# smyers119/sdrtrunk

Measured on NVIDIA B200. Metric: channelized+demodulated complex MS/s and real-time channel count at 1/2/4/8 GPU, higher is better.
Workload: dtype f32

## Files before the change

sdrtrunk_b200/csrc/filters.cu:

```cuda
#include <cstdint>

#include "filters.cuh"
#include "tma.cuh"

using namespace sdrgpu;

namespace {

__global__ void halfband_kernel(const float2 *__restrict__ in, long long in_stride, float2 *__restrict__ out,
                                long long out_stride, int out_off, int n_out, const __grid_constant__ HalfBandTaps taps)
{
    const int c = blockIdx.y;
    const float2 *x = in + (size_t)c * in_stride;
    float2 *y = out + (size_t)c * out_stride + out_off;
    const int L = taps.length, half = (L - 1) / 2;
    for (int m = blockIdx.x * blockDim.x + threadIdx.x; m < n_out; m += gridDim.x * blockDim.x) {
        const float2 *p = x + 2 * m;
        float ai = 0.0f, aq = 0.0f;
        for (int j = 0; j < half; j += 2) {
            const float2 a = p[j], b = p[L - 1 - j];
            const float h = taps.c[j];
            ai = __fadd_rn(ai, __fmul_rn(h, __fadd_rn(a.x, b.x)));
            aq = __fadd_rn(aq, __fmul_rn(h, __fadd_rn(a.y, b.y)));
        }
        const float2 mid = p[half];
        ai = __fadd_rn(ai, __fmul_rn(mid.x, 0.5f));
        aq = __fadd_rn(aq, __fmul_rn(mid.y, 0.5f));
        y[m] = make_float2(ai, aq);
    }
}

constexpr int kFirThreads = 128;
constexpr int kFirPer = 8;

__device__ __forceinline__ int skew8(int i) { return i + 2 * (i >> 3); }

__host__ __device__ inline int fir_window_len(int window) { return (window + 2 * (window >> 3) + 8 + 1) & ~1; }

__device__ __forceinline__ float agc_envelope(float i, float q)
{
    const float a = fabsf(i), b = fabsf(q);
    return (a > b) ? __fadd_rn(a, __fmul_rn(0.4f, b)) : __fadd_rn(b, __fmul_rn(0.4f, a));
}

__device__ __forceinline__ void load8p(const float2 *group, float2 *w)
{
    const float4 *p = reinterpret_cast<const float4 *>(group);
#pragma unroll
    for (int q = 0; q < 4; q++) {
        const float4 v = p[q];
        w[2 * q] = make_float2(v.x, v.y);
        w[2 * q + 1] = make_float2(v.z, v.w);
    }
}

__device__ __forceinline__ void cp_async16(void *dst_shared, const void *src_global)
{
    asm volatile("cp.async.cg.shared.global [%0], [%1], 16;" ::"r"((uint32_t)__cvta_generic_to_shared(dst_shared)), "l"(src_global) : "memory");
}
__device__ __forceinline__ void cp_async_commit() { asm volatile("cp.async.commit_group;" ::: "memory"); }
template <int kPending>
__device__ __forceinline__ void cp_async_wait() { asm volatile("cp.async.wait_group %0;" ::"n"(kPending) : "memory"); }

__device__ __forceinline__ void fir_taps8(const float2 *wbase, const float *hs, int kp, float2 (&acc)[kFirPer])
{
    float2 ga[8], gb[8], gc[8];
    load8p(wbase, gc);
    load8p(wbase - 10, gb);
#pragma unroll
    for (int j = 0; j < kFirPer; j++) acc[j] = make_float2(0.0f, 0.0f);
#define FIR_STEP(lo, hi, k0_)                                                                                   \
    {                                                                                                           \
        const float4 ha_ = *reinterpret_cast<const float4 *>(hs + (k0_));                                       \
        const float4 hb_ = *reinterpret_cast<const float4 *>(hs + (k0_) + 4);                                   \
        const float h_[8] = {ha_.x, ha_.y, ha_.z, ha_.w, hb_.x, hb_.y, hb_.z, hb_.w};                           \
        _Pragma("unroll") for (int u = 0; u < 8; u++) {                                                         \
            const float2 hh_ = make_float2(h_[u], h_[u]);                                                       \
            _Pragma("unroll") for (int j = 0; j < kFirPer; j++) {                                               \
                const float2 x_ = (j - u >= 0) ? hi[j - u] : lo[8 + j - u];                                     \
                acc[j] = __ffma2_rn(x_, hh_, acc[j]);                                                           \
            }                                                                                                   \
        }                                                                                                       \
    }
    int k0 = 0;
    for (; k0 + 24 <= kp; k0 += 24, wbase -= 30) {
        load8p(wbase - 20, ga);
        FIR_STEP(gb, gc, k0);
        load8p(wbase - 30, gc);
        FIR_STEP(ga, gb, k0 + 8);
        if (k0 + 24 < kp) load8p(wbase - 40, gb);
        FIR_STEP(gc, ga, k0 + 16);
    }
    if (k0 < kp) {
        if (k0 + 8 < kp) load8p(wbase - 20, ga);
        FIR_STEP(gb, gc, k0);
        if (k0 + 8 < kp) FIR_STEP(ga, gb, k0 + 8);
    }
#undef FIR_STEP
}

__global__ void __launch_bounds__(kFirThreads)
fir_agc_kernel(const float2 *__restrict__ in, long long in_stride, int in_off, float2 *__restrict__ out,
               long long out_stride, int tile, int n_total, int kp, float fir_gain, int agc, int tiles_per_cta,
               const __grid_constant__ FirTaps taps)
{
    extern __shared__ __align__(16) float2 xs_all[];
    __shared__ __align__(16) float hs[kMaxFirTaps];
    __shared__ float red[kFirThreads / 32];
    const int c = blockIdx.y, tid = threadIdx.x;
    const int window = kp + ((tile + 7) & ~7);
    const int wlen = fir_window_len(window);
    const int n_tiles = (n_total + tile - 1) / tile;
    const int first = blockIdx.x * tiles_per_cta, last = min(first + tiles_per_cta, n_tiles);
    const float2 *row = in + (size_t)c * in_stride + in_off;
    auto fill = [&](int blk, float2 *xs) {
        const float2 *src = row + (size_t)blk * tile - kp;
        const int valid = kp + min(tile, n_total - blk * tile);
        if (valid == window) {
            const float2 *s = src + 2 * tid;
            float2 *d = xs + skew8(2 * tid);
            for (int i = 2 * tid; i < window; i += 2 * kFirThreads, s += 2 * kFirThreads, d += 2 * kFirThreads + (kFirThreads >> 1))
                cp_async16(d, s);
        } else {
            for (int i = 2 * tid; i < window; i += 2 * kFirThreads) {
                float2 *dst = xs + skew8(i);
                if (i + 1 < valid) {
                    cp_async16(dst, src + i);
                } else {
                    dst[0] = i < valid ? src[i] : make_float2(0.f, 0.f);
                    dst[1] = make_float2(0.f, 0.f);
                }
            }
        }
        cp_async_commit();
    };
    for (int k = tid; k < kp; k += kFirThreads) hs[k] = taps.h[k];
    if (first < last) fill(first, xs_all);
    for (int blk = first; blk < last; blk++) {
    float2 *xs = xs_all + ((blk - first) & 1) * wlen;
    if (blk + 1 < last) {
        fill(blk + 1, xs_all + (((blk - first) & 1) ^ 1) * wlen);
        cp_async_wait<1>();
    } else {
        cp_async_wait<0>();
    }
    __syncthreads();
    const int block = min(tile, n_total - blk * tile);

    const int n0 = tid * kFirPer;
    float ai[kFirPer], aq[kFirPer];
    if (n0 < block) {
        const float2 *wbase = xs + skew8(kp + n0);
        if (kp > 0) {
            float2 acc[kFirPer];
            fir_taps8(wbase, hs, kp, acc);
#pragma unroll
            for (int j = 0; j < kFirPer; j++) {
                ai[j] = __fmul_rn(acc[j].x, fir_gain);
                aq[j] = __fmul_rn(acc[j].y, fir_gain);
            }
        } else {
            float2 x[kFirPer];
            load8p(wbase, x);
#pragma unroll
            for (int j = 0; j < kFirPer; j++) {
                ai[j] = x[j].x;
                aq[j] = x[j].y;
            }
        }
    } else {
#pragma unroll
        for (int j = 0; j < kFirPer; j++) {
            ai[j] = 0.0f;
            aq[j] = 0.0f;
        }
    }

    if (agc) {
        float m = 0.0001f;
#pragma unroll
        for (int j = 0; j < kFirPer; j++) {
            if (n0 + j < block) {
                const float env = agc_envelope(ai[j], aq[j]);
                if (env > m) m = env;
            }
        }
#pragma unroll
        for (int o = 16; o > 0; o >>= 1) m = fmaxf(m, __shfl_xor_sync(0xffffffffu, m, o));
        if ((tid & 31) == 0) red[tid >> 5] = m;
        __syncthreads();
        m = red[0];
#pragma unroll
        for (int wdx = 1; wdx < kFirThreads / 32; wdx++) m = fmaxf(m, red[wdx]);
        const float g = __fdiv_rn(1.0f, m);
#pragma unroll
        for (int j = 0; j < kFirPer; j++) {
            ai[j] = __fmul_rn(ai[j], g);
            aq[j] = __fmul_rn(aq[j], g);
        }
    }
    float2 *dst = out + (size_t)c * out_stride + (size_t)blk * tile + n0;
    if (n0 + kFirPer <= block && ((reinterpret_cast<uintptr_t>(dst) & 15) == 0)) {
#pragma unroll
        for (int j = 0; j < kFirPer; j += 2) *reinterpret_cast<float4 *>(dst + j) = make_float4(ai[j], aq[j], ai[j + 1], aq[j + 1]);
    } else {
#pragma unroll
        for (int j = 0; j < kFirPer; j++)
            if (n0 + j < block) dst[j] = make_float2(ai[j], aq[j]);
    }
    __syncthreads();
    }
}

constexpr int kSplitTile = 1024;
constexpr int kSplitPerWarp = kSplitTile / (kFirThreads / 32);

__device__ __forceinline__ void mbar_arrive(uint64_t *bar)
{
    asm volatile("mbarrier.arrive.shared::cta.b64 _, [%0];" ::"r"(tma::smem_addr(bar)) : "memory");
}

__global__ void __launch_bounds__(kFirThreads, 5)
fir_agc_split_kernel(const float2 *__restrict__ in, long long in_stride, int in_off, float2 *__restrict__ out,
                     long long out_stride, int n_tiles, int kp, float fir_gain, int tiles_per_cta,
                     const __grid_constant__ FirTaps taps)
{
    extern __shared__ __align__(16) float2 xs_all[];
    __shared__ __align__(16) float hs[kMaxFirTaps];
    __shared__ float red[2][kFirThreads / 32];
    __shared__ __align__(8) uint64_t bars[2];
    const int c = blockIdx.y, tid = threadIdx.x, warp = tid >> 5, lane = tid & 31;
    const int window = kp + kSplitPerWarp;
    const int wlen = fir_window_len(window);
    const int first = blockIdx.x * tiles_per_cta, last = min(first + tiles_per_cta, n_tiles);
    if (first >= last) return;
    for (int k = tid; k < kp; k += kFirThreads) hs[k] = taps.h[k];
    if (tid == 0) {
        tma::mbar_init(&bars[0], kFirThreads / 32);
        tma::mbar_init(&bars[1], kFirThreads / 32);
    }
    __syncthreads();
    float2 *xw = xs_all + (size_t)warp * 2 * wlen;
    const float2 *row = in + (size_t)c * in_stride + in_off + warp * kSplitPerWarp - kp;
    float2 *orow = out + (size_t)c * out_stride + warp * kSplitPerWarp + lane * kFirPer;
    auto fill = [&](int blk, float2 *xs) {
        const float2 *s = row + (size_t)blk * kSplitTile + 2 * lane;
        float2 *d = xs + skew8(2 * lane);
        for (int i = 2 * lane; i < window; i += 64, s += 64, d += 80) cp_async16(d, s);
        cp_async_commit();
    };
    const float2 *wfirst = xw + skew8(kp + lane * kFirPer);
    float pi[kFirPer], pq[kFirPer];
    auto finish = [&](int t) {
        const int p = t & 1;
        tma::mbar_wait(&bars[p], (uint32_t)((t >> 1) & 1));
        float m = red[p][0];
#pragma unroll
        for (int wdx = 1; wdx < kFirThreads / 32; wdx++) m = fmaxf(m, red[p][wdx]);
        const float g = __fdiv_rn(1.0f, m);
        float2 *dst = orow + (size_t)(first + t) * kSplitTile;
        if ((reinterpret_cast<uintptr_t>(dst) & 15) == 0) {
#pragma unroll
            for (int j = 0; j < kFirPer; j += 2)
                *reinterpret_cast<float4 *>(dst + j) = make_float4(__fmul_rn(pi[j], g), __fmul_rn(pq[j], g), __fmul_rn(pi[j + 1], g), __fmul_rn(pq[j + 1], g));
        } else {
#pragma unroll
            for (int j = 0; j < kFirPer; j++) dst[j] = make_float2(__fmul_rn(pi[j], g), __fmul_rn(pq[j], g));
        }
    };
    fill(first, xw);
    for (int blk = first; blk < last; blk++) {
        const int t = blk - first, p = t & 1;
        if (blk + 1 < last) {
            fill(blk + 1, xw + (p ^ 1) * wlen);
            cp_async_wait<1>();
        } else {
            cp_async_wait<0>();
        }
        __syncwarp();
        float2 acc[kFirPer];
        fir_taps8(wfirst + p * wlen, hs, kp, acc);
        float ai[kFirPer], aq[kFirPer];
        float m = 0.0001f;
#pragma unroll
        for (int j = 0; j < kFirPer; j++) {
            ai[j] = __fmul_rn(acc[j].x, fir_gain);
            aq[j] = __fmul_rn(acc[j].y, fir_gain);
            const float env = agc_envelope(ai[j], aq[j]);
            if (env > m) m = env;
        }
        m = __uint_as_float(__reduce_max_sync(0xffffffffu, __float_as_uint(m)));
        if (t > 0) finish(t - 1);
        if (lane == 0) {
            red[p][warp] = m;
            mbar_arrive(&bars[p]);
        }
#pragma unroll
        for (int j = 0; j < kFirPer; j++) {
            pi[j] = ai[j];
            pq[j] = aq[j];
        }
        __syncwarp();
    }
    finish(last - 1 - first);
}

constexpr int kFirTilesPerCta = 4;

}

namespace sdrgpu {

sdrgpu_status halfband_launch(const float2 *in, long long in_stride, float2 *out, long long out_stride, int out_off,
                              int n_out, int n_channels, const HalfBandTaps &taps, cudaStream_t stream)
{
    dim3 grid((n_out + 255) / 256 > 64 ? 64 : (n_out + 255) / 256, n_channels);
    halfband_kernel<<<grid, 256, 0, stream>>>(in - (taps.length - 1), in_stride, out, out_stride, out_off, n_out, taps);
    count_launch();
    SDRGPU_CUDA(cudaGetLastError());
    return SDRGPU_OK;
}

sdrgpu_status fir_agc_launch(const FirLaunch &a)
{
    const int kp = fir_padded_taps(a.n_taps);
    const int tile = a.agc_block > 0 ? a.agc_block : (a.n < 1024 ? a.n : 1024);
    const size_t smem_need = sizeof(float2) * 2 * (size_t)fir_window_len(kp + ((tile + 7) & ~7));
    const size_t smem = (a.throttle || g_tuning[SDRGPU_TUNE_THROTTLE_ALWAYS]) ? smem_for_ctas_per_sm(smem_need, sizeof(float) * (kMaxFirTaps + 8), g_tuning[SDRGPU_TUNE_FIR_CTAS_PER_SM]) : smem_need;
    if (smem > 48 * 1024) {
        static size_t fir_attr = 0;
        if (smem > fir_attr) {
            SDRGPU_CUDA(cudaFuncSetAttribute(fir_agc_kernel, cudaFuncAttributeMaxDynamicSharedMemorySize, 226 * 1024 - (int)(sizeof(float) * (kMaxFirTaps + 8))));
            fir_attr = 226 * 1024;
        }
    }
    const int n_tiles = (a.n + tile - 1) / tile;
    int tpc = (int)(((long long)a.n_channels * n_tiles) / (148 * 12));
    tpc = tpc < 1 ? 1 : (tpc > kFirTilesPerCta ? kFirTilesPerCta : tpc);
    if (g_tuning[SDRGPU_TUNE_FIR_TILES_PER_CTA] > 0) tpc = g_tuning[SDRGPU_TUNE_FIR_TILES_PER_CTA];
    if (tpc > n_tiles) tpc = n_tiles;
    dim3 grid((n_tiles + tpc - 1) / tpc, a.n_channels);
    const size_t split_smem = sizeof(float2) * 2 * (kFirThreads / 32) * (size_t)fir_window_len(kp + kSplitPerWarp);
    if (a.agc_block > 0 && tile == kSplitTile && a.n % kSplitTile == 0 && kp >= 8 && smem == smem_need &&
        split_smem <= 48 * 1024 && (a.in_off & 1) == 0) {
        fir_agc_split_kernel<<<grid, kFirThreads, split_smem, a.stream>>>(a.in, a.in_stride, a.in_off, a.out, a.out_stride,
                                                                          n_tiles, kp, a.gain, tpc, *a.taps);
    } else {
        fir_agc_kernel<<<grid, kFirThreads, smem, a.stream>>>(a.in, a.in_stride, a.in_off, a.out, a.out_stride, tile, a.n, kp,
                                                              a.gain, a.agc_block > 0, tpc, *a.taps);
    }
    count_launch();
    SDRGPU_CUDA(cudaGetLastError());
    return SDRGPU_OK;
}

}
```

Baseline: 27310.

## Compute 16 FIR outputs per thread in split AGC kernel with smem staging

Generalizes the FIR tap loop into a templated ring-buffered routine and has the split FIR+AGC kernel compute 16 outputs per thread, using 2 warps per CTA instead of 4. Computed outputs are parked in a swizzled shared-memory buffer instead of registers, and the taps move into dynamic shared memory. The goal is more register-level reuse of loaded samples per tap and lower per-CTA overhead, with coalesced float4 stores in the finish step. The costs are higher register pressure, fewer warps per CTA for latency hiding, and a changed 16-sample skew layout that must stay consistent with the fill logic.

```diff
diff --git a/sdrtrunk_b200/csrc/filters.cu b/sdrtrunk_b200/csrc/filters.cu
--- a/sdrtrunk_b200/csrc/filters.cu
+++ b/sdrtrunk_b200/csrc/filters.cu
@@ -34,6 +34,10 @@
 constexpr int kFirPer = 8;
 
 __device__ __forceinline__ int skew8(int i) { return i + 2 * (i >> 3); }
+__device__ __forceinline__ int skew16(int i) { return i + 2 * (i >> 4); }
+
+template <int kOut>
+__host__ __device__ constexpr int fir_group_offset(int a) { return -8 * a - 2 * ((8 * a + 2 * kOut - 1) / kOut - 1); }
 
 __host__ __device__ inline int fir_window_len(int window) { return (window + 2 * (window >> 3) + 8 + 1) & ~1; }
 
@@ -62,40 +66,55 @@
 template <int kPending>
 __device__ __forceinline__ void cp_async_wait() { asm volatile("cp.async.wait_group %0;" ::"n"(kPending) : "memory"); }
 
-__device__ __forceinline__ void fir_taps8(const float2 *wbase, const float *hs, int kp, float2 (&acc)[kFirPer])
-{
-    float2 ga[8], gb[8], gc[8];
-    load8p(wbase, gc);
-    load8p(wbase - 10, gb);
-#pragma unroll
-    for (int j = 0; j < kFirPer; j++) acc[j] = make_float2(0.0f, 0.0f);
-#define FIR_STEP(lo, hi, k0_)                                                                                   \
+template <int kOut>
+__device__ __forceinline__ void fir_taps(const float2 *wbase, const float *hs, int kp, float2 (&acc)[kOut])
+{
+    static_assert(kOut % 8 == 0, "whole groups of 8 outputs");
+    constexpr int kRing = kOut / 8 + 2;
+    static_assert(kRing <= 4, "at most 16 outputs per thread");
+    float2 g[kRing][8];
+#pragma unroll
+    for (int a = 1 - kOut / 8; a <= 1; a++) load8p(wbase + fir_group_offset<kOut>(a), g[(a + kRing) % kRing]);
+#pragma unroll
+    for (int j = 0; j < kOut; j++) acc[j] = make_float2(0.0f, 0.0f);
+#define FIR_STEP(i_, k0_)                                                                                       \
     {                                                                                                           \
         const float4 ha_ = *reinterpret_cast<const float4 *>(hs + (k0_));                                       \
         const float4 hb_ = *reinterpret_cast<const float4 *>(hs + (k0_) + 4);                                   \
         const float h_[8] = {ha_.x, ha_.y, ha_.z, ha_.w, hb_.x, hb_.y, hb_.z, hb_.w};                           \
         _Pragma("unroll") for (int u = 0; u < 8; u++) {                                                         \
             const float2 hh_ = make_float2(h_[u], h_[u]);                                                       \
-            _Pragma("unroll") for (int j = 0; j < kFirPer; j++) {                                               \
-                const float2 x_ = (j - u >= 0) ? hi[j - u] : lo[8 + j - u];                                     \
-                acc[j] = __ffma2_rn(x_, hh_, acc[j]);                                                           \
+            _Pragma("unroll") for (int j = 0; j < kOut; j++) {                                                  \
+                const int d_ = j - u + 8;                                                                       \
+                acc[j] = __ffma2_rn(g[((i_) + 1 - d_ / 8 + kRing) % kRing][d_ % 8], hh_, acc[j]);               \
             }                                                                                                   \
         }                                                                                                       \
     }
+#define RING_STEP(i_)                                                                                           \
+    if constexpr ((i_) < kRing) {                                                                               \
+        if ((i_) + 1 < kRing || k0 + 8 * kRing < kp) load8p(wbase + fir_group_offset<kOut>((i_) + 2), g[((i_) + 2) % kRing]);   \
+        FIR_STEP(i_, k0 + 8 * (i_));                                                                            \
+    }
     int k0 = 0;
-    for (; k0 + 24 <= kp; k0 += 24, wbase -= 30) {
-        load8p(wbase - 20, ga);
-        FIR_STEP(gb, gc, k0);
-        load8p(wbase - 30, gc);
-        FIR_STEP(ga, gb, k0 + 8);
-        if (k0 + 24 < kp) load8p(wbase - 40, gb);
-        FIR_STEP(gc, ga, k0 + 16);
+    static_assert(8 * kRing % kOut == 0, "whole blocks per turn");
+    for (; k0 + 8 * kRing <= kp; k0 += 8 * kRing, wbase += fir_group_offset<kOut>(kRing)) {
+        RING_STEP(0)
+        RING_STEP(1)
+        RING_STEP(2)
+        RING_STEP(3)
+    }
+#undef RING_STEP
+#define TAIL_STEP(i_, more_)                                                                                    \
+    if constexpr ((i_) < kRing - 1) {                                                                           \
+        const bool next_ = (i_) + 1 < kRing - 1 && k0 + 8 * ((i_) + 1) < kp;                                    \
+        if ((i_) + 2 < kRing && next_) load8p(wbase + fir_group_offset<kOut>((i_) + 2), g[((i_) + 2) % kRing]);                  \
+        FIR_STEP(i_, k0 + 8 * (i_));                                                                            \
+        if (next_) { more_ }                                                                                    \
     }
     if (k0 < kp) {
-        if (k0 + 8 < kp) load8p(wbase - 20, ga);
-        FIR_STEP(gb, gc, k0);
-        if (k0 + 8 < kp) FIR_STEP(ga, gb, k0 + 8);
-    }
+        TAIL_STEP(0, TAIL_STEP(1, TAIL_STEP(2, )))
+    }
+#undef TAIL_STEP
 #undef FIR_STEP
 }
 
@@ -153,7 +172,7 @@
         const float2 *wbase = xs + skew8(kp + n0);
         if (kp > 0) {
             float2 acc[kFirPer];
-            fir_taps8(wbase, hs, kp, acc);
+            fir_taps<kFirPer>(wbase, hs, kp, acc);
 #pragma unroll
             for (int j = 0; j < kFirPer; j++) {
                 ai[j] = __fmul_rn(acc[j].x, fir_gain);
@@ -213,59 +232,75 @@
 }
 
 constexpr int kSplitTile = 1024;
-constexpr int kSplitPerWarp = kSplitTile / (kFirThreads / 32);
+constexpr int kSplitPer = 16;
+constexpr int kSplitWarps = kSplitTile / (32 * kSplitPer);
+constexpr int kSplitThreads = 32 * kSplitWarps;
+constexpr int kSplitPerWarp = kSplitTile / kSplitWarps;
+
+__host__ __device__ inline int fir_split_window_len(int kp) { return (((kp + 15) & ~15) + kSplitPerWarp) / 16 * 18; }
+
+inline size_t fir_split_smem(int kp)
+{
+    return sizeof(float) * kp + sizeof(float2) * kSplitWarps * (2 * (size_t)fir_split_window_len(kp) + kSplitPerWarp);
+}
 
 __device__ __forceinline__ void mbar_arrive(uint64_t *bar)
 {
     asm volatile("mbarrier.arrive.shared::cta.b64 _, [%0];" ::"r"(tma::smem_addr(bar)) : "memory");
 }
 
-__global__ void __launch_bounds__(kFirThreads, 5)
+__global__ void __launch_bounds__(kSplitThreads, 6)
 fir_agc_split_kernel(const float2 *__restrict__ in, long long in_stride, int in_off, float2 *__restrict__ out,
                      long long out_stride, int n_tiles, int kp, float fir_gain, int tiles_per_cta,
                      const __grid_constant__ FirTaps taps)
 {
     extern __shared__ __align__(16) float2 xs_all[];
-    __shared__ __align__(16) float hs[kMaxFirTaps];
-    __shared__ float red[2][kFirThreads / 32];
+    __shared__ float red[2][kSplitWarps];
     __shared__ __align__(8) uint64_t bars[2];
     const int c = blockIdx.y, tid = threadIdx.x, warp = tid >> 5, lane = tid & 31;
     const int window = kp + kSplitPerWarp;
-    const int wlen = fir_window_len(window);
+    const int kp16 = (kp + 15) & ~15;
+    const int wlen = fir_split_window_len(kp);
     const int first = blockIdx.x * tiles_per_cta, last = min(first + tiles_per_cta, n_tiles);
     if (first >= last) return;
-    for (int k = tid; k < kp; k += kFirThreads) hs[k] = taps.h[k];
+    float *hs = reinterpret_cast<float *>(xs_all);
+    for (int k = tid; k < kp; k += kSplitThreads) hs[k] = taps.h[k];
     if (tid == 0) {
-        tma::mbar_init(&bars[0], kFirThreads / 32);
-        tma::mbar_init(&bars[1], kFirThreads / 32);
+        tma::mbar_init(&bars[0], kSplitWarps);
+        tma::mbar_init(&bars[1], kSplitWarps);
     }
     __syncthreads();
-    float2 *xw = xs_all + (size_t)warp * 2 * wlen;
+    float2 *xw = xs_all + kp / 2 + (size_t)warp * (2 * wlen + kSplitPerWarp);
+    float4 *park = reinterpret_cast<float4 *>(xw + 2 * wlen);
     const float2 *row = in + (size_t)c * in_stride + in_off + warp * kSplitPerWarp - kp;
-    float2 *orow = out + (size_t)c * out_stride + warp * kSplitPerWarp + lane * kFirPer;
+    float2 *orow = out + (size_t)c * out_stride + warp * kSplitPerWarp;
     auto fill = [&](int blk, float2 *xs) {
         const float2 *s = row + (size_t)blk * kSplitTile + 2 * lane;
-        float2 *d = xs + skew8(2 * lane);
-        for (int i = 2 * lane; i < window; i += 64, s += 64, d += 80) cp_async16(d, s);
+        float2 *d = xs + skew16(kp16 - kp + 2 * lane);
+        for (int i = 2 * lane; i < window; i += 64, s += 64, d += 72) cp_async16(d, s);
         cp_async_commit();
     };
-    const float2 *wfirst = xw + skew8(kp + lane * kFirPer);
-    float pi[kFirPer], pq[kFirPer];
+    const float2 *wfirst = xw + skew16(kp16 + lane * kSplitPer);
     auto finish = [&](int t) {
         const int p = t & 1;
         tma::mbar_wait(&bars[p], (uint32_t)((t >> 1) & 1));
         float m = red[p][0];
 #pragma unroll
-        for (int wdx = 1; wdx < kFirThreads / 32; wdx++) m = fmaxf(m, red[p][wdx]);
+        for (int wdx = 1; wdx < kSplitWarps; wdx++) m = fmaxf(m, red[p][wdx]);
         const float g = __fdiv_rn(1.0f, m);
         float2 *dst = orow + (size_t)(first + t) * kSplitTile;
-        if ((reinterpret_cast<uintptr_t>(dst) & 15) == 0) {
-#pragma unroll
-            for (int j = 0; j < kFirPer; j += 2)
-                *reinterpret_cast<float4 *>(dst + j) = make_float4(__fmul_rn(pi[j], g), __fmul_rn(pq[j], g), __fmul_rn(pi[j + 1], g), __fmul_rn(pq[j + 1], g));
-        } else {
-#pragma unroll
-            for (int j = 0; j < kFirPer; j++) dst[j] = make_float2(__fmul_rn(pi[j], g), __fmul_rn(pq[j], g));
+        const bool aligned = (reinterpret_cast<uintptr_t>(dst) & 15) == 0;
+#pragma unroll
+        for (int r = 0; r < kSplitPerWarp / 64; r++) {
+            const int w = 32 * r + lane;
+            const float4 v = park[(w & ~7) | ((w ^ (w >> 3)) & 7)];
+            const float4 y = make_float4(__fmul_rn(v.x, g), __fmul_rn(v.y, g), __fmul_rn(v.z, g), __fmul_rn(v.w, g));
+            if (aligned) {
+                reinterpret_cast<float4 *>(dst)[w] = y;
+            } else {
+                dst[2 * w] = make_float2(y.x, y.y);
+                dst[2 * w + 1] = make_float2(y.z, y.w);
+            }
         }
     };
     fill(first, xw);
@@ -278,15 +313,13 @@
             cp_async_wait<0>();
         }
         __syncwarp();
-        float2 acc[kFirPer];
-        fir_taps8(wfirst + p * wlen, hs, kp, acc);
-        float ai[kFirPer], aq[kFirPer];
+        float2 acc[kSplitPer];
+        fir_taps<kSplitPer>(wfirst + p * wlen, hs, kp, acc);
         float m = 0.0001f;
 #pragma unroll
-        for (int j = 0; j < kFirPer; j++) {
-            ai[j] = __fmul_rn(acc[j].x, fir_gain);
-            aq[j] = __fmul_rn(acc[j].y, fir_gain);
-            const float env = agc_envelope(ai[j], aq[j]);
+        for (int j = 0; j < kSplitPer; j++) {
+            acc[j] = make_float2(__fmul_rn(acc[j].x, fir_gain), __fmul_rn(acc[j].y, fir_gain));
+            const float env = agc_envelope(acc[j].x, acc[j].y);
             if (env > m) m = env;
         }
         m = __uint_as_float(__reduce_max_sync(0xffffffffu, __float_as_uint(m)));
@@ -295,11 +328,10 @@
             red[p][warp] = m;
             mbar_arrive(&bars[p]);
         }
-#pragma unroll
-        for (int j = 0; j < kFirPer; j++) {
-            pi[j] = ai[j];
-            pq[j] = aq[j];
-        }
+        __syncwarp();
+#pragma unroll
+        for (int q = 0; q < kSplitPer / 2; q++)
+            park[8 * lane + (q ^ (lane & 7))] = make_float4(acc[2 * q].x, acc[2 * q].y, acc[2 * q + 1].x, acc[2 * q + 1].y);
         __syncwarp();
     }
     finish(last - 1 - first);
@@ -340,11 +372,11 @@
     if (g_tuning[SDRGPU_TUNE_FIR_TILES_PER_CTA] > 0) tpc = g_tuning[SDRGPU_TUNE_FIR_TILES_PER_CTA];
     if (tpc > n_tiles) tpc = n_tiles;
     dim3 grid((n_tiles + tpc - 1) / tpc, a.n_channels);
-    const size_t split_smem = sizeof(float2) * 2 * (kFirThreads / 32) * (size_t)fir_window_len(kp + kSplitPerWarp);
+    const size_t split_smem = fir_split_smem(kp);
     if (a.agc_block > 0 && tile == kSplitTile && a.n % kSplitTile == 0 && kp >= 8 && smem == smem_need &&
         split_smem <= 48 * 1024 && (a.in_off & 1) == 0) {
-        fir_agc_split_kernel<<<grid, kFirThreads, split_smem, a.stream>>>(a.in, a.in_stride, a.in_off, a.out, a.out_stride,
-                                                                          n_tiles, kp, a.gain, tpc, *a.taps);
+        fir_agc_split_kernel<<<grid, kSplitThreads, split_smem, a.stream>>>(a.in, a.in_stride, a.in_off, a.out, a.out_stride,
+                                                                            n_tiles, kp, a.gain, tpc, *a.taps);
     } else {
         fir_agc_kernel<<<grid, kFirThreads, smem, a.stream>>>(a.in, a.in_stride, a.in_off, a.out, a.out_stride, tile, a.n, kp,
                                                               a.gain, a.agc_block > 0, tpc, *a.taps);
```

Result: no change. 27190, median of 6 (-0.4%).
